# chngdickson/ov2slam

Measured on AMD Instinct MI355X. Metric: tracked_frames_per_sec, higher is better.
Workload: dtype u8/s16 fixed-point + f32

## Files before the change

include/ov2slam_hip.h:

```cpp
#ifndef OV2SLAM_HIP_H
#define OV2SLAM_HIP_H

#include <stddef.h>
#include <stdint.h>

#ifdef __cplusplus
extern "C" {
#endif

typedef int ov2_status;
enum {
    OV2_OK = 0,
    OV2_ERR_INVALID = -1,
    OV2_ERR_HIP = -2,
    OV2_ERR_NOMEM = -3,
    OV2_ERR_NODEVICE = -4,
    OV2_ERR_UNSUPPORTED = -5
};

typedef struct ov2_ctx ov2_ctx;
typedef struct ov2_images ov2_images;
typedef struct ov2_pyr ov2_pyr;

ov2_status ov2_ctx_create(int device, ov2_ctx **out);
// ... 55 lines not shown
                            int max_iter, float eps, float err_th, float fb_th, int n, const float *kps_xy,
                            float *priors_xy, uint8_t *status);
ov2_status ov2_klt_track_fb_dev(ov2_ctx *ctx, const ov2_pyr *prev, const ov2_pyr *cur, int win, int nlevels,
                                int max_iter, float eps, float err_th, float fb_th, int n, const float *d_kps_xy,
                                float *d_priors_xy, uint8_t *d_status, const int32_t *d_img_idx,
                                uint32_t *d_iters);

ov2_status ov2_klt_tracking_frame_dev(ov2_ctx *ctx, const ov2_pyr *prev, const ov2_pyr *cur, int win,
                                      int nlevels_full, int max_iter, float eps, float err_th, float fb_th, int n,
                                      const float *d_kps_xy, const float *d_prior_xy, const uint8_t *d_has_prior,
                                      const int32_t *d_img_idx, float *d_out_xy, uint8_t *d_out_status,
                                      int32_t *d_p3p_req , uint32_t *d_iters );

ov2_status ov2_klt_set_lanes(ov2_ctx *ctx, int lanes);
ov2_status ov2_klt_set_stereo_split(ov2_ctx *ctx, int k);

ov2_status ov2_line_min_sad(ov2_ctx *ctx, const ov2_pyr *left, const ov2_pyr *right, int level, int nwinsize, int go_left,
                            int n, const float *pts_xy, float *xprior, float *l1err);
ov2_status ov2_line_min_sad_dev(ov2_ctx *ctx, const ov2_pyr *left, const ov2_pyr *right, int level, int nwinsize,
                                int go_left, int n, const float *d_pts_xy, const int32_t *d_img_idx, float *d_xprior,
                                float *d_l1err);

typedef struct ov2_cam_model {
    double K[4];
    int32_t model;
    int32_t n_coeffs;
    double D[5];
} ov2_cam_model;

ov2_status ov2_stereo_matching(ov2_ctx *ctx, const ov2_pyr *left, const ov2_pyr *right, int win, int nlevels_full,
// ... 539 lines not shown
```

ov2slam_amd/_lib.py:

```python
import ctypes as C
import os

_HERE = os.path.dirname(os.path.abspath(__file__))
LIB_PATH = os.environ.get("OV2SLAM_HIP_LIB") or os.path.join(_HERE, "lib", "libov2hip.so")

vp = C.c_void_p
vpp = C.POINTER(C.c_void_p)
ip = C.POINTER(C.c_int)
fp = C.POINTER(C.c_float)

SIGNATURES = {
    "ov2_ctx_create": (C.c_int, [C.c_int, vpp]),
    "ov2_ctx_create_ex": (C.c_int, [C.c_int, C.c_int, vpp]),
    "ov2_ctx_destroy": (None, [vp]),
    "ov2_last_error": (C.c_char_p, [vp]),
    "ov2_status_string": (C.c_char_p, [C.c_int]),
    "ov2_ctx_synchronize": (C.c_int, [vp]),
    "ov2_ctx_set_kf_overlap": (C.c_int, [vp, C.c_int]),
    "ov2_ctx_set_kf_lazy_join": (C.c_int, [vp, C.c_int]),
    "ov2_ctx_get_kf_lazy_join": (C.c_int, [vp]),
    "ov2_ctx_kf_join_stats": (C.c_int, [vp, C.POINTER(C.c_int64)]),
    "ov2_kf_ranges_independent": (C.c_int, [C.POINTER(C.c_size_t), C.c_int, C.POINTER(C.c_size_t), C.c_int,
                                            C.POINTER(C.c_size_t), C.c_int, C.POINTER(C.c_size_t), C.c_int]),
    "ov2_ctx_set_wave_prio": (C.c_int, [vp, C.c_int]),
# ... 25 lines not shown
    "ov2_pyr_retain": (None, [vp]),
    "ov2_pyr_release": (None, [vp]),
    "ov2_pyr_release_from": (None, [vp, vp]),
    "ov2_pyr_batch": (C.c_int, [vp]),
    "ov2_pyr_nlevels": (C.c_int, [vp]),
    "ov2_pyr_level_size": (C.c_int, [vp, C.c_int, ip, ip, ip]),
    "ov2_pyr_download_level": (C.c_int, [vp, vp, C.c_int, C.c_int, vp, vp]),
    "ov2_klt_track_fb": (C.c_int, [vp, vp, vp, C.c_int, C.c_int, C.c_int, C.c_float, C.c_float, C.c_float,
                                   C.c_int, vp, vp, vp]),
    "ov2_klt_track_fb_dev": (C.c_int, [vp, vp, vp, C.c_int, C.c_int, C.c_int, C.c_float, C.c_float, C.c_float,
                                       C.c_int, vp, vp, vp, vp, vp]),
    "ov2_klt_tracking_frame_dev": (C.c_int, [vp, vp, vp, C.c_int, C.c_int, C.c_int, C.c_float, C.c_float,
                                             C.c_float, C.c_int, vp, vp, vp, vp, vp, vp, vp, vp]),
    "ov2_klt_set_lanes": (C.c_int, [vp, C.c_int]),
    "ov2_klt_set_stereo_split": (C.c_int, [vp, C.c_int]),
    "ov2_line_min_sad": (C.c_int, [vp, vp, vp, C.c_int, C.c_int, C.c_int, C.c_int, vp, vp, vp]),
    "ov2_line_min_sad_dev": (C.c_int, [vp, vp, vp, C.c_int, C.c_int, C.c_int, C.c_int, vp, vp, vp, vp]),
    "ov2_stereo_matching": (C.c_int, [vp, vp, vp, C.c_int, C.c_int, C.c_int, C.c_float, C.c_float, C.c_float, C.c_int,
                                      vp, vp, vp, vp, C.c_int, vp, vp, vp, vp]),
    "ov2_stereo_matching_dev": (C.c_int, [vp, vp, vp, C.c_int, C.c_int, C.c_int, C.c_float, C.c_float, C.c_float, C.c_int,
                                          vp, vp, vp, vp, vp, C.c_int, vp, vp, vp, vp, vp]),
    "ov2_detect_grid": (C.c_int, [vp, vp, C.c_int, C.c_int, C.c_int, C.POINTER(C.c_double), C.c_int, vp, vp, C.c_int, ip, vp]),
    "ov2_detect_grid_batch": (C.c_int, [vp, vp, C.c_int, C.c_int, C.POINTER(C.c_double), ip, vp, vp, C.c_int, ip, vp, C.c_int]),
    "ov2_detect_grid_batch_dev": (C.c_int, [vp, vp, C.c_int, C.c_int, vp, C.c_int, vp, vp, vp, vp, C.c_int, vp, vp, C.c_int]),
    "ov2_fast_detect_batch": (C.c_int, [vp, vp, C.c_int, C.c_int, vp, vp, C.c_int, C.c_int, vp, vp, vp, vp]),
    "ov2_fast_detect_batch_dev": (C.c_int, [vp, vp, C.c_int, C.c_int, C.c_int, vp, vp, C.c_int, C.c_int, vp, vp, vp, vp]),
    "ov2_ba_default_options": (None, [vp, C.c_float]),
    "ov2_ba_solve": (C.c_int, [vp, vp, vp, vp]),
    "ov2_ba_solve_batch": (C.c_int, [vp, C.c_int, vp, vp, vp]),
    "ov2_ba_solve_batch_dev": (C.c_int, [vp, C.c_int, vp, vp, vp]),
# ... 120 lines not shown
```

ov2slam_amd/csrc/ctx.hip:

```cpp
#include "ov2_internal.h"

#include <cstdlib>

ov2_status ov2_set_err(ov2_ctx *ctx, ov2_status s, const char *fmt, ...)
{
    char buf[512];
    va_list ap;
    va_start(ap, fmt);
    vsnprintf(buf, sizeof(buf), fmt, ap);
    va_end(ap);
    if (ctx) {
        std::lock_guard<std::mutex> g(ctx->mu);
        ctx->err = buf;
    }
    return s;
}

extern "C" const char *ov2_status_string(ov2_status s)
{
    switch (s) {
    case OV2_OK: return "ok";
    case OV2_ERR_INVALID: return "invalid argument";
    case OV2_ERR_HIP: return "HIP runtime error";
    case OV2_ERR_NOMEM: return "out of memory";
// ... 99 lines not shown
        for (int x = 0; x < OV2_CU_MASK_XCDS; ++x) {
            int bits = 0, own = 0;
            for (int k = x; k < total; k += OV2_CU_MASK_XCDS, ++own) bits += (int)(mask[k >> 5] >> (k & 31) & 1u);
            effective_cus += bits ? bits : own;
        }
    }
    ov2_ctx *c = new ov2_ctx();
    c->device = device;
    c->scratch_dev = nullptr;
    c->scratch_bytes = 0;
    c->tmp_img = nullptr;
    c->ktime_on = false;
    c->wave_prio = high_priority ? OV2_WAVE_PRIO_HIGH : 0;
    c->klt_lanes = 0;
    c->klt_stereo_split = -1;
    c->knn_lanes = 0;
    c->knn_cus = effective_cus;
    c->cu_share = n_cus;
    c->cu_layout = layout;
    c->counts_as_high = false;
    c->lcd_splits = 0;
    c->lcd_calls = 0;
    c->ba_arena = nullptr;
    c->ba_arena_cap = 0;
    c->ba_host = nullptr;
    c->ba_host_cap = 0;
    c->ba_copy_stream = nullptr;
    c->klt_counts[0] = c->klt_counts[1] = nullptr;
    c->klt_counts_words = 0;
    c->klt_counts_cur = 0;
// ... 555 lines not shown
```

ov2slam_amd/csrc/klt.hip:

```cpp
#include <cstdlib>

#include "ov2_internal.h"
#include "ov2_wave.h"

using namespace ov2wave;

namespace {

struct klt_params {
    int win, nlevels, max_iter;
    int wave_prio;
    double eps2;
    float err_th;
    double fb_th;
    float min_eig_thr;
    int rule33;
};

#define W_BITS 14

__device__ __forceinline__ void lk_weights(float a, float b, int &w00, int &w01, int &w10, int &w11)
{
    w00 = (int)__builtin_rintf((1.f - a) * (1.f - b) * (float)(1 << W_BITS));
    w01 = (int)__builtin_rintf(a * (1.f - b) * (float)(1 << W_BITS));
    w10 = (int)__builtin_rintf((1.f - a) * b * (float)(1 << W_BITS));
    w11 = (1 << W_BITS) - w00 - w01 - w10;
}

__device__ __forceinline__ unsigned ld_u16(const unsigned char *p)
{
    unsigned short r;
    __builtin_memcpy(&r, p, 2);
// ... 423 lines not shown
    }
}
template <int B, int NB>
__device__ __forceinline__ void klt3_stage_region(const level_ptrs &J, int rr0, int cc0, int c, bool store, unsigned char *lj)
{
    if constexpr (B < NB) {
        constexpr int T0 = klt3::NLD * B / NB, T1 = klt3::NLD * (B + 1) / NB;
        klt3_segs<T0, T1> S;
        klt3_load_region(J, rr0, cc0, c, S);
        klt3_store_region(S, c, store, lj);
        __builtin_amdgcn_sched_barrier(0);
        klt3_stage_region<B + 1, NB>(J, rr0, cc0, c, store, lj);
    }
}

template <int WIN>
__device__ __forceinline__ int lk_level3(const level_ptrs &I, const level_ptrs &J, int pad, int level, int max_level,
                                         bool run, float kx, float ky, float &nx_io, float &ny_io, int &status,
                                         float &err, const klt_params &P, int c, bool lane_ok, unsigned &passes,
                                         unsigned char *lj)
{
    static_assert(WIN == 9, "three lanes x three columns");
#ifdef KLT3_VGPR_CLAIM
    asm volatile("" ::: KLT3_VGPR_CLAIM);
#endif
    constexpr int NPX = 3 * WIN, NQ = (NPX + 1) / 2;
    const float FLT_SCALE = 1.f / (float)(1 << 20);
    const float half = (float)(WIN - 1) * 0.5f;
    const float lscale = __builtin_ldexpf(1.f, -level);
    float px = kx * lscale, py = ky * lscale;
    float nx, ny;
    if (level == max_level) { nx = nx_io * lscale; ny = ny_io * lscale; }
    else { nx = nx_io * 2.f; ny = ny_io * 2.f; }
    if (run) { nx_io = nx; ny_io = ny; }

    px -= half; py -= half;
    const int ipx = (int)floorf(px), ipy = (int)floorf(py);
    if (run && (ipx < -WIN || ipx >= I.w || ipy < -WIN || ipy >= I.h)) {
        if (level == 0) { status = 0; err = 0.f; }
        run = false;
    }
    if (!__any(run)) return 0;
    if (run) passes += 1u;
    int w00, w01, w10, w11;
    lk_weights(px - (float)ipx, py - (float)ipy, w00, w01, w10, w11);

    unsigned Iv2[NQ], Ix2[NQ], Iy2[NQ];
    int sA11 = 0, sA12 = 0, sA22 = 0;
    int rr0, cc0;
    {
        const float sx = nx - half, sy = ny - half;
        const int inx0 = (int)floorf(sx), iny0 = (int)floorf(sy);
        const bool in0 = run && !(inx0 < -WIN || inx0 >= J.w || iny0 < -WIN || iny0 >= J.h);
        klt3_region_origin(J, pad, in0 ? inx0 : 0, in0 ? iny0 : 0, rr0, cc0);
        const int bx0 = (run ? (OV2_LM + ipx) : OV2_LM) + 3 * c, by = run ? (ipy + pad) : pad;
        const int ax = bx0 - 1;
        const unsigned io = I.img_o + (unsigned)(by * I.istride + (ax & ~3));
        const unsigned shI = (unsigned)ax & 3u;
        struct row3 { unsigned x, y, z; };
        row3 irow[WIN + 3];
#define KLT3_LOAD_ROW(p)                                                                                                  \
    do {                                                                                                                  \
        const int dr = (p) == 0 ? (by > 0 ? -1 : 0) : ((p) == WIN + 2 ? (by + WIN + 1 < I.rows ? WIN + 1 : WIN) : (p) - 1); \
        __builtin_memcpy(&irow[p], __builtin_assume_aligned(I.base + (size_t)(io + (unsigned)(dr * I.istride)), 4), 12);   \
    } while (0)
        constexpr int R1 = 6;
// ... 89 lines not shown
    float D = A11 * A22 - A12 * A12;
    const float min_eig = __fdiv_rn(A22 + A11 - __fsqrt_rn((A11 - A22) * (A11 - A22) + 4.f * A12 * A12),
                                    (float)(2 * WIN * WIN));
    if (run) {
        err = min_eig;
        if (min_eig < P.min_eig_thr || D < 1.1920929e-07f ) {
            if (level == 0) status = 0;
            run = false;
        }
    }
    D = __fdiv_rn(1.f, D);

    nx -= half; ny -= half;
    float pdx = 0.f, pdy = 0.f;
    int iters = 0;
    for (int j = 0; j < P.max_iter; ++j) {
        if (!__any(run)) break;
        const int inx = (int)floorf(nx), iny = (int)floorf(ny);
        if (run && (inx < -WIN || inx >= J.w || iny < -WIN || iny >= J.h)) {
            if (level == 0) status = 0;
            run = false;
        }
        int w00j, w01j, w10j, w11j;
        lk_weights(nx - (float)inx, ny - (float)iny, w00j, w01j, w10j, w11j);
        int rb = run ? iny + pad - rr0 : 0, cb = run ? OV2_LM + inx - cc0 : 0;
        const bool out = (unsigned)rb > (unsigned)klt3::ROW_SPAN || (unsigned)cb > (unsigned)klt3::COL_SPAN;
        if (__any(out)) {
            __syncthreads();
            if (out) {
                klt3_region_origin(J, pad, inx, iny, rr0, cc0);
                klt3_stage_region<0, KLT3_REGION_BATCHES>(J, rr0, cc0, c, lane_ok, lj);
                rb = iny + pad - rr0; cb = OV2_LM + inx - cc0;
// ... 34 lines not shown
        float b1, b2;
        if (__all((unsigned)(pb1 + (1 << 27)) < (1u << 28) && (unsigned)(pb2 + (1 << 27)) < (1u << 28))) {
            b1 = (float)sum3_i32(pb1, c) * FLT_SCALE;
            b2 = (float)sum3_i32(pb2, c) * FLT_SCALE;
        } else {
            b1 = (float)sum3_f64((double)pb1, c) * FLT_SCALE;
            b2 = (float)sum3_f64((double)pb2, c) * FLT_SCALE;
        }
        const float dx = (A12 * b2 - A22 * b1) * D;
        const float dy = (A12 * b1 - A11 * b2) * D;
        if (run) {
            ++iters;
            nx += dx; ny += dy;
            nx_io = nx + half; ny_io = ny + half;
            if ((double)dx * dx + (double)dy * dy <= P.eps2) run = false;
            else if (j > 0 && fabsf(dx + pdx) <= 0.01f && fabsf(dy + pdy) <= 0.01f) {
                nx_io -= dx * 0.5f; ny_io -= dy * 0.5f;
                run = false;
            }
            pdx = dx; pdy = dy;
        }
    }
    return iters;
}

template <int WIN, int GL>
__device__ __forceinline__ int lk_pass(const level_ptrs &I, const level_ptrs &J, int pad, int level, int max_level, bool run,
                                       float kx, float ky, float &nx_io, float &ny_io, int &status, float &err,
                                       const klt_params &P, int sub, bool lane_ok, unsigned &passes, unsigned char *smem, int slot)
{
    if constexpr (GL == 3) {
        return lk_level3<WIN>(I, J, pad, level, max_level, run, kx, ky, nx_io, ny_io, status, err, P, sub, lane_ok, passes,
                              smem + slot * klt3::RSZ);
    } else {
        constexpr int KPW = 64 / GL, WB = klt_lds<WIN>::WB, GB = klt_lds<WIN>::GB;
        return lk_level<WIN, GL>(I, J, pad, level, max_level, run, kx, ky, nx_io, ny_io, status, err, P, sub, passes,
                                 smem + slot * WB, smem + KPW * WB + slot * WB, smem + 2 * KPW * WB + slot * GB);
    }
}

struct __attribute__((aligned(16))) klt_handover { float fx, fy, err; unsigned work; };

template <int WIN, int GL>
__device__ __forceinline__ int fb_track(const ov2_pyr_view &pv, const ov2_pyr_view &cv, int b, bool act, float kx,
                                          float ky, float &fx, float &fy, const klt_params &P, int nlevels, int sub,
                                          bool lane_ok, unsigned &work, unsigned char *smem, int slot,
                                          int l_hi, int l_lo, float err0, unsigned work0, float &err_out)
{
    int status = 1;
    float err = err0;
    unsigned it = work0 & 0xffffu, passes = work0 >> 16;
    for (int l = l_hi; l >= l_lo; --l) {
        const level_ptrs I = level_of(pv, l, b), J = level_of(cv, l, b);
        it += lk_pass<WIN, GL>(I, J, pv.pad, l, nlevels, act, kx, ky, fx, fy, status, err, P, sub, lane_ok, passes, smem, slot);
    }
    if (l_lo > 0) {
        work = it | (passes << 16);
        err_out = err;
        return 0;
    }
    const int W0 = cv.lv[0].w, H0 = cv.lv[0].h;
    int ok = act && status && !(err > P.err_th) &&
             (1.f <= fx && fx < (float)W0 - 1.f && 1.f <= fy && fy < (float)H0 - 1.f);
    int st2 = 1;
    float e2 = 0.f, bx = kx, by = ky;
    {
        const level_ptrs I = level_of(cv, 0, b), J = level_of(pv, 0, b);
        it += lk_pass<WIN, GL>(I, J, cv.pad, 0, 0, ok != 0, fx, fy, bx, by, st2, e2, P, sub, lane_ok, passes, smem, slot);
    }
    if (ok) {
        if (!st2) ok = 0;
        else {
            const float dx = kx - bx, dy = ky - by;
            const double nrm = __dsqrt_rn((double)dx * dx + (double)dy * dy);
            if (nrm > P.fb_th) ok = 0;
        }
    }
    work = it | (passes << 16);
    return ok;
}

template <int WIN, int GL>
__device__ __forceinline__ int fb_track(const ov2_pyr_view &pv, const ov2_pyr_view &cv, int b, bool act, float kx,
                                          float ky, float &fx, float &fy, const klt_params &P, int nlevels, int sub,
                                          bool lane_ok, unsigned &work, unsigned char *smem, int slot)
{
    float err;
    return fb_track<WIN, GL>(pv, cv, b, act, kx, ky, fx, fy, P, nlevels, sub, lane_ok, work, smem, slot, nlevels, 0, 0.f, 0u, err);
}

#define KLT_GL8_MIN_KPS 65536
#ifndef KLT_STEREO_SPLIT_DEFAULT
#define KLT_STEREO_SPLIT_DEFAULT 0
#endif
#ifndef KLT_SPLIT_C_FIRST
#define KLT_SPLIT_C_FIRST 1
#endif
#ifndef KLT_WAVE_CAP
#define KLT_WAVE_CAP 4
#endif
#ifndef KLT3_WAVE_MIN
#define KLT3_WAVE_MIN 2
#endif
#define KLT_WAVES(W, G) ((G) == 3 ? KLT3_WAVE_MIN : 1), ((G) == 3 ? KLT3_WAVES : KLT_WAVE_CAP)

template <int WIN, int KLT_GL>
__global__ __launch_bounds__(64) __attribute__((amdgpu_waves_per_eu(KLT_WAVES(WIN, KLT_GL)))) void klt_fb_kernel(ov2_pyr_view pv, ov2_pyr_view cv, klt_params P, int n,
                                                    const float2 *__restrict__ kps, float2 *__restrict__ priors,
// ... 80 lines not shown
        out_status[i] = (unsigned char)ok;
        if (iters) iters[is_a ? i : n + i] = work;
        if (is_a) atomicAdd(&counts[64 * b + (i & 63)], 1u + ((unsigned)ok << 16));
    }
    const bool retry = mine && is_a && !ok;
    const unsigned long long rm = __ballot(retry);
    if (rm) {
        const int lane = (int)threadIdx.x, leader = __ffsll((long long)rm) - 1;
        int base = 0;
        if (lane == leader) base = (int)atomicAdd(&cnt[2], (unsigned)__popcll(rm));
        base = __shfl(base, leader);
        if (retry) list_c[base + __popcll(rm & ((1ull << lane) - 1ull))] = i;
    }
}

template <int WIN, int KLT_GL, bool SPLIT>
__global__ __launch_bounds__(64) __attribute__((amdgpu_waves_per_eu(KLT_WAVES(WIN, KLT_GL)))) void klt_stage1_kernel(ov2_pyr_view pv, ov2_pyr_view cv, klt_params P, int n,
                                                        const float2 *__restrict__ kps,
                                                        const float2 *__restrict__ prior,
                                                        const int *__restrict__ img_idx, float2 *__restrict__ out_xy,
                                                        unsigned char *__restrict__ out_status,
                                                        unsigned *__restrict__ counts ,
                                                        unsigned *__restrict__ iters, const int *__restrict__ list_a,
                                                        const int *__restrict__ list_b, unsigned *__restrict__ cnt,
                                                        int *__restrict__ list_c,
                                                        int b_word ,
                                                        int split_k ,
                                                        klt_handover *__restrict__ hand )
{
    __shared__ __attribute__((aligned(16))) unsigned char smem[klt_smem<WIN, KLT_GL>::BYTES];
    using M = klt_map<KLT_GL>;
// ... 4 lines not shown
    const int g = is_a ? (int)blockIdx.x - groups_b : (int)blockIdx.x;
    const int total = is_a ? total_a : total_b;
    if (g * KLT_KPW >= total) return;
    ov2wave::set_wave_prio(P.wave_prio);
    const int slot = M::slot((int)threadIdx.x), sub = M::sub((int)threadIdx.x), idx = g * KLT_KPW + slot;
    const bool lane_ok = M::lane_ok((int)threadIdx.x);
    const bool act = idx < total && lane_ok;
    const int i = (is_a ? list_a : list_b)[idx < total ? idx : total - 1];
    const float2 kp = kps[i];
    const int b = img_idx ? img_idx[i] : 0;
    float2 pr = (is_a || !P.rule33) ? prior[i] : kp;
    unsigned work = 0;
    const int nl = is_a ? min(1, pv.nlevels - 1) : P.nlevels;
    const bool upper = SPLIT && !is_a;
    float err;
    const int ok = fb_track<WIN, KLT_GL>(pv, cv, b, act, kp.x, kp.y, pr.x, pr.y, P, nl, sub, lane_ok, work, smem, slot, nl,
                                         upper ? split_k + 1 : 0, 0.f, 0u, err);
    if (upper) {
        if (act && sub == 0) hand[i] = klt_handover{pr.x, pr.y, err, work};
        return;
    }
    klt_stage1_finish(act && sub == 0, is_a, i, b, n, ok, pr, work, out_xy, out_status, counts, iters, cnt, list_c);
}

template <int WIN, int KLT_GL>
__global__ __launch_bounds__(64) __attribute__((amdgpu_waves_per_eu(KLT_WAVES(WIN, KLT_GL)))) void klt_stage2_kernel(ov2_pyr_view pv, ov2_pyr_view cv, klt_params P, int n,
                                                        const float2 *__restrict__ kps,
                                                        const int *__restrict__ img_idx, float2 *__restrict__ out_xy,
                                                        unsigned char *__restrict__ out_status,
                                                        const unsigned *__restrict__ counts, int *__restrict__ p3p_req,
                                                        unsigned *__restrict__ iters, const int *__restrict__ list_c,
                                                        const unsigned *__restrict__ cnt, int batch,
                                                        unsigned *__restrict__ next_counts, int next_words,
                                                        const int *__restrict__ list_b, int b_word,
                                                        const float2 *__restrict__ prior,
                                                        int split_k ,
                                                        const klt_handover *__restrict__ hand)
{
    __shared__ __attribute__((aligned(16))) unsigned char smem[klt_smem<WIN, KLT_GL>::BYTES];
    using M = klt_map<KLT_GL>;
    constexpr int KLT_KPW = M::KPW;
    const int slot = M::slot((int)threadIdx.x), sub = M::sub((int)threadIdx.x);
    const bool lane_ok = M::lane_ok((int)threadIdx.x);
    for (int q = blockIdx.x * 64 + threadIdx.x; q < next_words; q += gridDim.x * 64) next_counts[q] = 0u;
    auto tally = [&](int b, int &n3, int &good) {
        n3 = 0; good = 0;
        if constexpr (KLT_GL == 3) {
            for (int q = sub; q < 64; q += 3) {
                const unsigned cw = counts[64 * b + q];
                n3 += (int)(cw & 0xffffu); good += (int)(cw >> 16);
            }
            n3 = sum3_i32(n3, sub); good = sum3_i32(good, sub);
        } else {
            for (int q = 0; q < 64 / KLT_GL; ++q) {
                const unsigned cw = counts[64 * b + sub * (64 / KLT_GL) + q];
                n3 += (int)(cw & 0xffffu); good += (int)(cw >> 16);
            }
            n3 = row_sum_i32<KLT_GL>(n3); good = row_sum_i32<KLT_GL>(good);
        }
    };
    if (p3p_req && P.rule33) {
        for (int b0 = blockIdx.x * KLT_KPW; b0 < batch; b0 += gridDim.x * KLT_KPW) {
            const int b = b0 + slot;
            int n3, good;
            tally(min(b, batch - 1), n3, good);
            if (b < batch && lane_ok && sub == 0 && n3 > 0 && (double)good < 0.33 * (double)n3) p3p_req[b] = 1;
        }
    }
    const int total_b = (int)cnt[b_word], total_c = (int)cnt[2];
    const bool b_first = split_k < 0 || !KLT_SPLIT_C_FIRST;
    const int groups_1 = ((b_first ? total_b : total_c) + KLT_KPW - 1) / KLT_KPW;
    const bool first = (int)blockIdx.x < groups_1;
    const bool is_b = first == b_first;
    const int g = first ? (int)blockIdx.x : (int)blockIdx.x - groups_1;
    const int total = is_b ? total_b : total_c;
    if (g * KLT_KPW >= total) return;
    ov2wave::set_wave_prio(P.wave_prio);
    const int idx = g * KLT_KPW + slot;
    const bool act = idx < total && lane_ok;
    const int i = (is_b ? list_b : list_c)[idx < total ? idx : total - 1];
    const int b = img_idx ? img_idx[i] : 0;
    const float2 kp = kps[i];
    float2 pr;
    int l_hi = P.nlevels;
    float err0 = 0.f;
    unsigned work0 = 0;
    if (is_b) {
        if (split_k >= 0) {
            const klt_handover hr = hand[i];
            pr = make_float2(hr.fx, hr.fy);
            err0 = hr.err; work0 = hr.work; l_hi = split_k;
        } else {
            pr = prior[i];
        }
    } else {
        int n3, good;
        tally(b, n3, good);
        const bool drop = P.rule33 && n3 > 0 && (double)good < 0.33 * (double)n3;
        pr = drop ? kp : out_xy[i];
    }
    unsigned work = 0;
    float err;
    const int ok = fb_track<WIN, KLT_GL>(pv, cv, b, act, kp.x, kp.y, pr.x, pr.y, P, P.nlevels, sub, lane_ok, work, smem, slot,
                                         l_hi, 0, err0, work0, err);
    if (act && sub == 0) {
        out_xy[i] = pr;
        out_status[i] = (unsigned char)ok;
        if (iters) iters[n + i] = work;
    }
}

int klt_lanes_for(const ov2_ctx *c, int n, int win, const ov2_pyr *a, const ov2_pyr *b)
{
    static const int env = [] { const char *e = getenv("OV2_KLT_LANES"); return e ? atoi(e) : 0; }();
    const int forced = c->klt_lanes ? c->klt_lanes : env;
    const bool fits32 = a->buf->bytes < (1ull << 32) && b->buf->bytes < (1ull << 32);
    if (forced == 8 || forced == 16 || (forced == 3 && win == 9 && fits32)) return forced;
    if (win == 9 && fits32) return 3;
    return n >= KLT_GL8_MIN_KPS ? 8 : 16;
// ... 11 lines not shown
        return ov2_set_err(c, OV2_ERR_INVALID, "win=%d unsupported (odd, 3..11, <= pyramid pad %d)", win, a.pad);
    if (nlevels < 0) return ov2_set_err(c, OV2_ERR_INVALID, "nlevels < 0");
    if (a.nlevels < nlevels + 1) nlevels = a.nlevels - 1;
    P->win = win;
    P->wave_prio = c->wave_prio;
    P->nlevels = nlevels;
    P->max_iter = max_iter < 0 ? 0 : (max_iter > 100 ? 100 : max_iter);
    double e = (double)eps;
    if (e < 0.) e = 0.;
    if (e > 10.) e = 10.;
    P->eps2 = e * e;
    P->err_th = err_th;
    P->fb_th = (double)fb_th;
    P->min_eig_thr = 1e-4f;
    P->rule33 = 1;
    return OV2_OK;
}

}

extern "C" ov2_status ov2_klt_set_lanes(ov2_ctx *c, int lanes)
{
    if (!c) return OV2_ERR_INVALID;
    if (lanes != 0 && lanes != 3 && lanes != 8 && lanes != 16) return ov2_set_err(c, OV2_ERR_INVALID, "lanes per keypoint: 0 (auto), 3, 8 or 16");
    c->klt_lanes = lanes;
    return OV2_OK;
}

extern "C" ov2_status ov2_klt_set_stereo_split(ov2_ctx *c, int k)
{
    if (!c) return OV2_ERR_INVALID;
    c->klt_stereo_split = k < 0 ? -1 : k;
    return OV2_OK;
}

extern "C" ov2_status ov2_klt_track_fb_dev(ov2_ctx *c, const ov2_pyr *prev, const ov2_pyr *cur, int win, int nlevels,
                                           int max_iter, float eps, float err_th, float fb_th, int n,
                                           const float *d_kps, float *d_priors, uint8_t *d_status,
                                           const int32_t *d_img_idx, uint32_t *d_iters)
{
    if (!c) return OV2_ERR_INVALID;
    if (n == 0) return OV2_OK;
    if (n < 0 || !d_kps || !d_priors || !d_status) return ov2_set_err(c, OV2_ERR_INVALID, "null/negative argument");
    klt_params P;
    ov2_status s = make_params(c, prev, cur, win, nlevels, max_iter, eps, err_th, fb_th, &P);
    if (s != OV2_OK) return s;
    OV2_HIP(c, hipSetDevice(c->device));
// ... 68 lines not shown
    if (n == 0) return OV2_OK;
    if (n < 0 || !d_kps || !d_prior || !d_has_prior || !d_out_xy || !d_out_status)
        return ov2_set_err(c, OV2_ERR_INVALID, "null/negative argument");
    klt_params P;
    ov2_status s = make_params(c, prev, cur, win, nlevels_full, max_iter, eps, err_th, fb_th, &P);
    if (s != OV2_OK) return s;
    P.rule33 = rule33 ? 1 : 0;
    OV2_HIP(c, hipSetDevice(c->device));
    if ((s = ov2_pyr_wait_ready(c, prev)) != OV2_OK || (s = ov2_pyr_wait_ready(c, cur)) != OV2_OK) return s;
    const int lanes = klt_lanes_for(c, n, win, prev, cur);
    if (lanes != 3 && ((s = ov2_pyr_need_grad(c, prev)) != OV2_OK || (s = ov2_pyr_need_grad(c, cur)) != OV2_OK)) return s;
    const int B = prev->buf->batch;
    const size_t cnt_words = (size_t)B * 64 + 16;
    if (cnt_words > c->klt_counts_words) {
        OV2_HIP(c, hipStreamSynchronize(c->stream));
        for (int i = 0; i < 2; ++i) {
            if (c->klt_counts[i]) OV2_HIP(c, hipFree(c->klt_counts[i]));
            c->klt_counts[i] = nullptr;
        }
        c->klt_counts_words = 0;
        const size_t words = cnt_words + cnt_words / 2;
        for (int i = 0; i < 2; ++i) OV2_HIP(c, hipMalloc((void **)&c->klt_counts[i], words * sizeof(unsigned)));
        c->klt_counts_words = words;
        c->klt_counts_dirty = true;
    }
    if (c->klt_counts_dirty)
        for (int i = 0; i < 2; ++i) OV2_HIP(c, hipMemsetAsync(c->klt_counts[i], 0, c->klt_counts_words * sizeof(unsigned), c->stream));
    c->klt_counts_dirty = true;
    void *scr = nullptr;
    const size_t lists_bytes = (3 * (size_t)n * sizeof(int) + 255) / 256 * 256;
    s = ov2_scratch(c, lists_bytes + (size_t)n * sizeof(klt_handover) + 256, &scr);
    if (s != OV2_OK) return s;
    unsigned *counts = c->klt_counts[c->klt_counts_cur], *live_cnt = counts + (size_t)B * 64;
    unsigned *next_counts = c->klt_counts[c->klt_counts_cur ^ 1];
    const int next_words = (int)c->klt_counts_words;
    int *list_a = (int *)scr, *list_b = list_a + n, *list_c = list_b + n;
    const size_t N = (size_t)n;
    const ov2_byte_range kf_rd[4] = {ov2_range(d_kps, 8 * N), ov2_range(d_prior, 8 * N), ov2_range(d_has_prior, N), ov2_range(d_img_idx, 4 * N)};
    const ov2_byte_range kf_wr[4] = {ov2_range(d_out_xy, 8 * N), ov2_range(d_out_status, N), ov2_range(d_p3p_req, sizeof(int32_t) * (size_t)B),
                                     ov2_range(d_iters, 8 * N)};
    const hipStream_t ms = ov2_kf_stream_for(c, true, kf_rd, 4, kf_wr, 4);
    if (c->kf.want_stereo_ev) {
        OV2_HIP(c, hipEventRecord(c->kf.fork, c->stream.h));
        c->kf.want_stereo_ev = false;
    }
    const dim3 cgrid((n + KLT_COMPACT_KPWG - 1) / KLT_COMPACT_KPWG);
    const int want_k = c->klt_stereo_split < 0 ? KLT_STEREO_SPLIT_DEFAULT : c->klt_stereo_split;
    const int split_k = (!P.rule33 && want_k < P.nlevels) ? want_k : -1;
    const int b_word1 = (P.rule33 || split_k >= 0) ? 1 : 3, b_word2 = P.rule33 ? 3 : 1;
    klt_handover *hand = reinterpret_cast<klt_handover *>((char *)scr + lists_bytes);
#define KLT_STAGES_GL(W, G)                                                                                     \
    do {                                                                                                        \
         \
        const dim3 tgrid((n + klt_map<G>::KPW - 1) / klt_map<G>::KPW + 2);                                      \
        OV2_LAUNCH_ON(c, OV2_K_DETECT + 4, ms, klt_compact_kernel, cgrid, dim3(256), 0, ms, n, d_has_prior,     \
                   d_iters, list_a, list_b, live_cnt, d_p3p_req, B, P.wave_prio);                               \
        if (split_k >= 0)                                                                                       \
            OV2_LAUNCH_ON(c, OV2_K_KLT_STAGE1, ms, (klt_stage1_kernel<W, G, true>), tgrid, dim3(64), 0, ms,     \
                       prev->buf->view, cur->buf->view, P, n, reinterpret_cast<const float2 *>(d_kps),          \
                       reinterpret_cast<const float2 *>(d_prior), d_img_idx, reinterpret_cast<float2 *>(d_out_xy), \
                       d_out_status, counts, d_iters, list_a, list_b, live_cnt, list_c, b_word1, split_k, hand); \
        else                                                                                                    \
            OV2_LAUNCH_ON(c, OV2_K_KLT_STAGE1, ms, (klt_stage1_kernel<W, G, false>), tgrid, dim3(64), 0, ms,    \
                       prev->buf->view, cur->buf->view, P, n, reinterpret_cast<const float2 *>(d_kps),          \
                       reinterpret_cast<const float2 *>(d_prior), d_img_idx, reinterpret_cast<float2 *>(d_out_xy), \
                       d_out_status, counts, d_iters, list_a, list_b, live_cnt, list_c, b_word1, split_k, hand); \
        OV2_LAUNCH_ON(c, OV2_K_KLT_STAGE2, ms, (klt_stage2_kernel<W, G>), tgrid, dim3(64), 0, ms,               \
                   prev->buf->view, cur->buf->view, P, n, reinterpret_cast<const float2 *>(d_kps), d_img_idx,   \
                   reinterpret_cast<float2 *>(d_out_xy), d_out_status, counts, d_p3p_req, d_iters, list_c,      \
                   live_cnt, B, next_counts, next_words, list_b, b_word2,                                       \
                   reinterpret_cast<const float2 *>(d_prior), split_k, hand);                                   \
    } while (0)
#define KLT_STAGES(W)                                                                                           \
    do {                                                                                                        \
        if (lanes == 8) KLT_STAGES_GL(W, 8);                                                                       \
        else KLT_STAGES_GL(W, 16);                                                                              \
    } while (0)
    switch (win) {
    case 3: KLT_STAGES(3); break;
    case 5: KLT_STAGES(5); break;
    case 7: KLT_STAGES(7); break;
    case 9:
        if (lanes == 3) KLT_STAGES_GL(9, 3);
        else KLT_STAGES(9);
        break;
    default: KLT_STAGES(11); break;
    }
#undef KLT_STAGES
#undef KLT_STAGES_GL
    OV2_HIP(c, hipGetLastError());
    c->klt_counts_cur ^= 1;
    c->klt_counts_dirty = false;
    return OV2_OK;
}
```

ov2slam_amd/csrc/ov2_internal.h:

```cpp
#pragma once
#include <hip/hip_runtime.h>

#include <atomic>
#include <cstdarg>
#include <cstdio>
#include <cstring>
#include <mutex>
#include <string>
#include <vector>

#include "../../include/ov2slam_hip.h"

#define OV2_MAX_LEVELS 8
#define OV2_LM 16

struct ov2_level_desc {
    int w, h;
    int istride;
    int gstride;
    int rows;
    size_t img_off;
    size_t grad_off;
    size_t img_bstride;
    size_t grad_bstride;
// ... 154 lines not shown
    void *lpg_dev;
    size_t lpg_dev_cap;
    void *ba_arena2;
    size_t ba_arena2_cap;
    void *ba_host;
    size_t ba_host_cap;
    unsigned *klt_counts[2];
    size_t klt_counts_words;
    int klt_counts_cur;
    bool klt_counts_dirty;
    hipStream_t ba_copy_stream;
    hipEvent_t ba_copy_ev[2];
    int wave_prio;
    int klt_lanes;
    int klt_stereo_split;
    int knn_lanes;
    int knn_cus;
    int cu_share, cu_layout;
    bool counts_as_high;
    int lcd_splits;
    long long lcd_calls;
    std::vector<struct ov2_lcd_table *> lcd_tables;
    bool ktime_on;
    std::vector<ov2_ktime_rec> ktime_recs;
    std::vector<hipEvent_t> ktime_free;
};

struct ov2_images {
    ov2_ctx *ctx;
    int batch, w, h;
// ... 54 lines not shown
```

ov2slam_amd/frontend.py:

```python
import ctypes as C

import numpy as np

from . import _lib


WAVE_PRIO_HIGH = 2


CU_LAYOUT_SPREAD, CU_LAYOUT_PACKED = 0, 1
CU_MASK_XCDS = 8


def cu_mask_build(total_cus, n_cus, layout=CU_LAYOUT_SPREAD):
    out = (C.c_uint32 * ((int(total_cus) + 31) // 32 if total_cus > 0 else 1))()
    st = _lib.load().ov2_cu_mask_build(int(total_cus), int(n_cus), int(layout), out)
    if st != 0:
        raise _lib.Ov2Error(f"ov2_cu_mask_build({total_cus}, {n_cus}, {layout}): status {st}")
    return np.array(out, np.uint32)


def _check(ctx_handle, status):
    if status != 0:
        lib = _lib.load()
# ... 19 lines not shown
        self.h = h

    def close(self):
        if getattr(self, "h", None):
            self.lib.ov2_ctx_destroy(self.h)
            self.h = None

    def __del__(self):
        self.close()

    def set_klt_lanes(self, lanes):
        _check(self.h, self.lib.ov2_klt_set_lanes(self.h, int(lanes)))

    def set_stereo_split(self, k):
        _check(self.h, self.lib.ov2_klt_set_stereo_split(self.h, int(k)))

    def set_knn_lanes(self, lanes):
        _check(self.h, self.lib.ov2_knn_set_lanes(self.h, int(lanes)))

    def set_kf_overlap(self, on):
        _check(self.h, self.lib.ov2_ctx_set_kf_overlap(self.h, int(bool(on))))

    def set_wave_prio(self, level):
        _check(self.h, self.lib.ov2_ctx_set_wave_prio(self.h, int(level)))

    def get_wave_prio(self):
        return int(self.lib.ov2_ctx_get_wave_prio(self.h))

    def get_cu_share(self):
        return int(self.lib.ov2_ctx_get_cu_share(self.h))
# ... 361 lines not shown
```

Baseline: 309,500.

## Park straggler KLT lanes in split stereo descent and resume them compacted

In the split two-stage KLT path, a wave whose live keypoint count drops to a threshold after k iterations saves each lane's iteration state to a park record. Those keypoints are appended to a new compacted list, and stage 2 launches extra 'D' waves that resume them at the saved level and iteration. The aim is to stop nearly empty waves from running long Lucas-Kanade tails at low occupancy. In exchange it adds per-keypoint park records, atomics, extra stage-2 groups and per-level park counters, plus an env knob and stats API.

```diff
diff --git a/include/ov2slam_hip.h b/include/ov2slam_hip.h
--- a/include/ov2slam_hip.h
+++ b/include/ov2slam_hip.h
@@ -93,6 +93,8 @@
 
 ov2_status ov2_klt_set_lanes(ov2_ctx *ctx, int lanes);
 ov2_status ov2_klt_set_stereo_split(ov2_ctx *ctx, int k);
+ov2_status ov2_klt_set_stereo_park(ov2_ctx *ctx, int k, int t);
+ov2_status ov2_ctx_klt_park_stats(ov2_ctx *ctx, int64_t out[10]);
 
 ov2_status ov2_line_min_sad(ov2_ctx *ctx, const ov2_pyr *left, const ov2_pyr *right, int level, int nwinsize, int go_left,
                             int n, const float *pts_xy, float *xprior, float *l1err);
diff --git a/ov2slam_amd/_lib.py b/ov2slam_amd/_lib.py
--- a/ov2slam_amd/_lib.py
+++ b/ov2slam_amd/_lib.py
@@ -63,6 +63,8 @@
                                              C.c_float, C.c_int, vp, vp, vp, vp, vp, vp, vp, vp]),
     "ov2_klt_set_lanes": (C.c_int, [vp, C.c_int]),
     "ov2_klt_set_stereo_split": (C.c_int, [vp, C.c_int]),
+    "ov2_klt_set_stereo_park": (C.c_int, [vp, C.c_int, C.c_int]),
+    "ov2_ctx_klt_park_stats": (C.c_int, [vp, C.POINTER(C.c_int64)]),
     "ov2_line_min_sad": (C.c_int, [vp, vp, vp, C.c_int, C.c_int, C.c_int, C.c_int, vp, vp, vp]),
     "ov2_line_min_sad_dev": (C.c_int, [vp, vp, vp, C.c_int, C.c_int, C.c_int, C.c_int, vp, vp, vp, vp]),
     "ov2_stereo_matching": (C.c_int, [vp, vp, vp, C.c_int, C.c_int, C.c_int, C.c_float, C.c_float, C.c_float, C.c_int,
diff --git a/ov2slam_amd/csrc/ctx.hip b/ov2slam_amd/csrc/ctx.hip
--- a/ov2slam_amd/csrc/ctx.hip
+++ b/ov2slam_amd/csrc/ctx.hip
@@ -137,6 +137,17 @@
     c->wave_prio = high_priority ? OV2_WAVE_PRIO_HIGH : 0;
     c->klt_lanes = 0;
     c->klt_stereo_split = -1;
+    c->klt_park_k = c->klt_park_t = -1;
+    if (const char *park_env = getenv("OV2_KLT_STEREO_PARK")) {
+        int k = -1, t = -1;
+        const int got = sscanf(park_env, "%d,%d", &k, &t);
+        if (got >= 1 && !(k > 0 && got == 2 && t == 0)) {
+            c->klt_park_k = k < 0 ? -1 : (k > 100 ? 100 : k);
+            c->klt_park_t = (k < 0 || got < 2 || t < 0) ? -1 : (t > 21 ? 21 : t);
+        }
+    }
+    for (auto &v : c->klt_park_folded) v = 0;
+    c->klt_park_calls = 0;
     c->knn_lanes = 0;
     c->knn_cus = effective_cus;
     c->cu_share = n_cus;
diff --git a/ov2slam_amd/csrc/klt.hip b/ov2slam_amd/csrc/klt.hip
--- a/ov2slam_amd/csrc/klt.hip
+++ b/ov2slam_amd/csrc/klt.hip
@@ -12,10 +12,13 @@
     int wave_prio;
     double eps2;
     float err_th;
+    short park_k, park_t;
     double fb_th;
     float min_eig_thr;
     int rule33;
 };
+
+static_assert(sizeof(klt_params) == 48, "klt_params: the kernels' argument layout");
 
 #define W_BITS 14
 
@@ -469,11 +472,34 @@
     }
 }
 
-template <int WIN>
+struct __attribute__((aligned(8))) klt_park_rec {
+    float nx, ny;
+    float nx_io, ny_io;
+    float pdx, pdy;
+    float err;
+    unsigned work;
+    int level, j;
+};
+#define KLT_HAND_PARKED 0xffffffffu
+#define KLT_CNT_D 4
+#define KLT_CNT_PARKED 8
+#define KLT_PARK_WORDS 16
+static_assert(OV2_MAX_LEVELS + 1 <= KLT_PARK_WORDS, "parked per level + D waves");
+static_assert(KLT_CNT_PARKED + OV2_MAX_LEVELS <= 16, "the list-length block has 16 words");
+struct klt_park_io {
+    klt_park_rec *rec;
+    unsigned *level_cnt;
+    unsigned it;
+    int level;
+    bool on;
+    bool parked;
+};
+
+template <int WIN, int PM = 0>
 __device__ __forceinline__ int lk_level3(const level_ptrs &I, const level_ptrs &J, int pad, int level, int max_level,
                                          bool run, float kx, float ky, float &nx_io, float &ny_io, int &status,
                                          float &err, const klt_params &P, int c, bool lane_ok, unsigned &passes,
-                                         unsigned char *lj)
+                                         unsigned char *lj, klt_park_io &pk)
 {
     static_assert(WIN == 9, "three lanes x three columns");
 #ifdef KLT3_VGPR_CLAIM
@@ -487,7 +513,9 @@
     float nx, ny;
     if (level == max_level) { nx = nx_io * lscale; ny = ny_io * lscale; }
     else { nx = nx_io * 2.f; ny = ny_io * 2.f; }
-    if (run) { nx_io = nx; ny_io = ny; }
+    bool res = false;
+    if constexpr (PM == 2) res = run && level == pk.level;
+    if (run && !res) { nx_io = nx; ny_io = ny; }
 
     px -= half; py -= half;
     const int ipx = (int)floorf(px), ipy = (int)floorf(py);
@@ -496,7 +524,7 @@
         run = false;
     }
     if (!__any(run)) return 0;
-    if (run) passes += 1u;
+    if (run && !res) passes += 1u;
     int w00, w01, w10, w11;
     lk_weights(px - (float)ipx, py - (float)ipy, w00, w01, w10, w11);
 
@@ -504,7 +532,10 @@
     int sA11 = 0, sA12 = 0, sA22 = 0;
     int rr0, cc0;
     {
-        const float sx = nx - half, sy = ny - half;
+        float sx = nx - half, sy = ny - half;
+        if constexpr (PM == 2) {
+            if (res) { sx = pk.rec->nx; sy = pk.rec->ny; }
+        }
         const int inx0 = (int)floorf(sx), iny0 = (int)floorf(sy);
         const bool in0 = run && !(inx0 < -WIN || inx0 >= J.w || iny0 < -WIN || iny0 >= J.h);
         klt3_region_origin(J, pad, in0 ? inx0 : 0, in0 ? iny0 : 0, rr0, cc0);
@@ -624,8 +655,32 @@
     nx -= half; ny -= half;
     float pdx = 0.f, pdy = 0.f;
     int iters = 0;
+    int j0 = 0;
+    if constexpr (PM == 2) {
+        if (res) {
+            const klt_park_rec r = *pk.rec;
+            nx = r.nx; ny = r.ny; pdx = r.pdx; pdy = r.pdy; j0 = r.j;
+        }
+    }
     for (int j = 0; j < P.max_iter; ++j) {
+        if constexpr (PM == 2) {
+            if (j + j0 >= P.max_iter) run = false;
+        }
         if (!__any(run)) break;
+        if constexpr (PM == 1) {
+            if (pk.on && j >= (int)P.park_k) {
+                const unsigned long long live = __ballot(run && c == 0 && lane_ok);
+                if (__popcll(live) <= (int)P.park_t) {
+                    if (run) {
+                        if (c == 0)
+                            *pk.rec = klt_park_rec{nx, ny, nx_io, ny_io, pdx, pdy, err, (pk.it + (unsigned)iters) | (passes << 16), level, j};
+                        pk.parked = true;
+                    }
+                    if ((int)threadIdx.x == __ffsll((long long)live) - 1) atomicAdd(&pk.level_cnt[level], (unsigned)__popcll(live));
+                    break;
+                }
+            }
+        }
         const int inx = (int)floorf(nx), iny = (int)floorf(ny);
         if (run && (inx < -WIN || inx >= J.w || iny < -WIN || iny >= J.h)) {
             if (level == 0) status = 0;
@@ -690,7 +745,7 @@
             nx += dx; ny += dy;
             nx_io = nx + half; ny_io = ny + half;
             if ((double)dx * dx + (double)dy * dy <= P.eps2) run = false;
-            else if (j > 0 && fabsf(dx + pdx) <= 0.01f && fabsf(dy + pdy) <= 0.01f) {
+            else if ((PM == 2 ? j + j0 : j) > 0 && fabsf(dx + pdx) <= 0.01f && fabsf(dy + pdy) <= 0.01f) {
                 nx_io -= dx * 0.5f; ny_io -= dy * 0.5f;
                 run = false;
             }
@@ -700,15 +755,17 @@
     return iters;
 }
 
-template <int WIN, int GL>
+template <int WIN, int GL, int PM = 0>
 __device__ __forceinline__ int lk_pass(const level_ptrs &I, const level_ptrs &J, int pad, int level, int max_level, bool run,
                                        float kx, float ky, float &nx_io, float &ny_io, int &status, float &err,
-                                       const klt_params &P, int sub, bool lane_ok, unsigned &passes, unsigned char *smem, int slot)
+                                       const klt_params &P, int sub, bool lane_ok, unsigned &passes, unsigned char *smem, int slot,
+                                       klt_park_io &pk)
 {
     if constexpr (GL == 3) {
-        return lk_level3<WIN>(I, J, pad, level, max_level, run, kx, ky, nx_io, ny_io, status, err, P, sub, lane_ok, passes,
-                              smem + slot * klt3::RSZ);
+        return lk_level3<WIN, PM>(I, J, pad, level, max_level, run, kx, ky, nx_io, ny_io, status, err, P, sub, lane_ok, passes,
+                                  smem + slot * klt3::RSZ, pk);
     } else {
+        static_assert(PM == 0, "parking is the three-lane mapping's");
         constexpr int KPW = 64 / GL, WB = klt_lds<WIN>::WB, GB = klt_lds<WIN>::GB;
         return lk_level<WIN, GL>(I, J, pad, level, max_level, run, kx, ky, nx_io, ny_io, status, err, P, sub, passes,
                                  smem + slot * WB, smem + KPW * WB + slot * WB, smem + 2 * KPW * WB + slot * GB);
@@ -717,18 +774,22 @@
 
 struct __attribute__((aligned(16))) klt_handover { float fx, fy, err; unsigned work; };
 
-template <int WIN, int GL>
+template <int WIN, int GL, int PM = 0>
 __device__ __forceinline__ int fb_track(const ov2_pyr_view &pv, const ov2_pyr_view &cv, int b, bool act, float kx,
                                           float ky, float &fx, float &fy, const klt_params &P, int nlevels, int sub,
                                           bool lane_ok, unsigned &work, unsigned char *smem, int slot,
-                                          int l_hi, int l_lo, float err0, unsigned work0, float &err_out)
+                                          int l_hi, int l_lo, float err0, unsigned work0, float &err_out, klt_park_io &pk)
 {
     int status = 1;
     float err = err0;
     unsigned it = work0 & 0xffffu, passes = work0 >> 16;
+    klt_park_io none{};
     for (int l = l_hi; l >= l_lo; --l) {
         const level_ptrs I = level_of(pv, l, b), J = level_of(cv, l, b);
-        it += lk_pass<WIN, GL>(I, J, pv.pad, l, nlevels, act, kx, ky, fx, fy, status, err, P, sub, lane_ok, passes, smem, slot);
+        bool run = act;
+        if constexpr (PM == 1) { run = act && !pk.parked; pk.it = it; }
+        if constexpr (PM == 2) run = act && (pk.level < 0 || l <= pk.level);
+        it += lk_pass<WIN, GL, PM>(I, J, pv.pad, l, nlevels, run, kx, ky, fx, fy, status, err, P, sub, lane_ok, passes, smem, slot, pk);
     }
     if (l_lo > 0) {
         work = it | (passes << 16);
@@ -742,7 +803,7 @@
     float e2 = 0.f, bx = kx, by = ky;
     {
         const level_ptrs I = level_of(cv, 0, b), J = level_of(pv, 0, b);
-        it += lk_pass<WIN, GL>(I, J, cv.pad, 0, 0, ok != 0, fx, fy, bx, by, st2, e2, P, sub, lane_ok, passes, smem, slot);
+        it += lk_pass<WIN, GL>(I, J, cv.pad, 0, 0, ok != 0, fx, fy, bx, by, st2, e2, P, sub, lane_ok, passes, smem, slot, none);
     }
     if (ok) {
         if (!st2) ok = 0;
@@ -762,12 +823,19 @@
                                           bool lane_ok, unsigned &work, unsigned char *smem, int slot)
 {
     float err;
-    return fb_track<WIN, GL>(pv, cv, b, act, kx, ky, fx, fy, P, nlevels, sub, lane_ok, work, smem, slot, nlevels, 0, 0.f, 0u, err);
+    klt_park_io none{};
+    return fb_track<WIN, GL>(pv, cv, b, act, kx, ky, fx, fy, P, nlevels, sub, lane_ok, work, smem, slot, nlevels, 0, 0.f, 0u, err, none);
 }
 
 #define KLT_GL8_MIN_KPS 65536
 #ifndef KLT_STEREO_SPLIT_DEFAULT
 #define KLT_STEREO_SPLIT_DEFAULT 0
+#endif
+#ifndef KLT_STEREO_PARK_K_DEFAULT
+#define KLT_STEREO_PARK_K_DEFAULT 4
+#endif
+#ifndef KLT_STEREO_PARK_T_DEFAULT
+#define KLT_STEREO_PARK_T_DEFAULT 4
 #endif
 #ifndef KLT_SPLIT_C_FIRST
 #define KLT_SPLIT_C_FIRST 1
@@ -878,7 +946,7 @@
     }
 }
 
-template <int WIN, int KLT_GL, bool SPLIT>
+template <int WIN, int KLT_GL, bool SPLIT, bool PARK = false>
 __global__ __launch_bounds__(64) __attribute__((amdgpu_waves_per_eu(KLT_WAVES(WIN, KLT_GL)))) void klt_stage1_kernel(ov2_pyr_view pv, ov2_pyr_view cv, klt_params P, int n,
                                                         const float2 *__restrict__ kps,
                                                         const float2 *__restrict__ prior,
@@ -913,16 +981,36 @@
     const int nl = is_a ? min(1, pv.nlevels - 1) : P.nlevels;
     const bool upper = SPLIT && !is_a;
     float err;
-    const int ok = fb_track<WIN, KLT_GL>(pv, cv, b, act, kp.x, kp.y, pr.x, pr.y, P, nl, sub, lane_ok, work, smem, slot, nl,
-                                         upper ? split_k + 1 : 0, 0.f, 0u, err);
+    klt_park_io pk{};
+    if constexpr (PARK) {
+        static_assert(SPLIT && KLT_GL == 3, "parking belongs to the split descent of the three-lane mapping");
+        pk.rec = reinterpret_cast<klt_park_rec *>(hand + n) + i;
+        pk.level_cnt = cnt + KLT_CNT_PARKED;
+        pk.on = upper && P.park_k > 0;
+    }
+    const int ok = fb_track<WIN, KLT_GL, PARK ? 1 : 0>(pv, cv, b, act, kp.x, kp.y, pr.x, pr.y, P, nl, sub, lane_ok, work, smem, slot, nl,
+                                                       upper ? split_k + 1 : 0, 0.f, 0u, err, pk);
     if (upper) {
-        if (act && sub == 0) hand[i] = klt_handover{pr.x, pr.y, err, work};
+        if constexpr (PARK) {
+            const bool mine = act && sub == 0;
+            if (mine) hand[i] = klt_handover{pr.x, pr.y, err, pk.parked ? KLT_HAND_PARKED : work};
+            const unsigned long long dm = __ballot(mine && pk.parked);
+            if (dm) {
+                const int lane = (int)threadIdx.x, leader = __ffsll((long long)dm) - 1;
+                int base = 0;
+                if (lane == leader) base = (int)atomicAdd(&cnt[KLT_CNT_D], (unsigned)__popcll(dm));
+                base = __shfl(base, leader);
+                if (mine && pk.parked) (list_c + n)[base + __popcll(dm & ((1ull << lane) - 1ull))] = i;
+            }
+        } else {
+            if (act && sub == 0) hand[i] = klt_handover{pr.x, pr.y, err, work};
+        }
         return;
     }
     klt_stage1_finish(act && sub == 0, is_a, i, b, n, ok, pr, work, out_xy, out_status, counts, iters, cnt, list_c);
 }
 
-template <int WIN, int KLT_GL>
+template <int WIN, int KLT_GL, bool PARK = false>
 __global__ __launch_bounds__(64) __attribute__((amdgpu_waves_per_eu(KLT_WAVES(WIN, KLT_GL)))) void klt_stage2_kernel(ov2_pyr_view pv, ov2_pyr_view cv, klt_params P, int n,
                                                         const float2 *__restrict__ kps,
                                                         const int *__restrict__ img_idx, float2 *__restrict__ out_xy,
@@ -941,6 +1029,14 @@
     constexpr int KLT_KPW = M::KPW;
     const int slot = M::slot((int)threadIdx.x), sub = M::sub((int)threadIdx.x);
     const bool lane_ok = M::lane_ok((int)threadIdx.x);
+    if constexpr (PARK) {
+        static_assert(KLT_GL == 3, "parking belongs to the three-lane mapping");
+        if (blockIdx.x == 0 && threadIdx.x <= OV2_MAX_LEVELS) {
+            const int q = (int)threadIdx.x;
+            const unsigned v = q < OV2_MAX_LEVELS ? cnt[KLT_CNT_PARKED + q] : (cnt[KLT_CNT_D] + KLT_KPW - 1) / KLT_KPW;
+            if (v) atomicAdd(&next_counts[next_words + q], v);
+        }
+    }
     for (int q = blockIdx.x * 64 + threadIdx.x; q < next_words; q += gridDim.x * 64) next_counts[q] = 0u;
     auto tally = [&](int b, int &n3, int &good) {
         n3 = 0; good = 0;
@@ -967,28 +1063,48 @@
         }
     }
     const int total_b = (int)cnt[b_word], total_c = (int)cnt[2];
-    const bool b_first = split_k < 0 || !KLT_SPLIT_C_FIRST;
-    const int groups_1 = ((b_first ? total_b : total_c) + KLT_KPW - 1) / KLT_KPW;
-    const bool first = (int)blockIdx.x < groups_1;
-    const bool is_b = first == b_first;
-    const int g = first ? (int)blockIdx.x : (int)blockIdx.x - groups_1;
-    const int total = is_b ? total_b : total_c;
+    bool is_b, is_d = false;
+    int g, total;
+    if constexpr (PARK) {
+        const int total_d = (int)cnt[KLT_CNT_D];
+        const int groups_c = (total_c + KLT_KPW - 1) / KLT_KPW, groups_d = (total_d + KLT_KPW - 1) / KLT_KPW;
+        const int bid = (int)blockIdx.x;
+        is_d = bid >= groups_c && bid < groups_c + groups_d;
+        is_b = bid >= groups_c + groups_d;
+        g = is_b ? bid - groups_c - groups_d : (is_d ? bid - groups_c : bid);
+        total = is_b ? total_b : (is_d ? total_d : total_c);
+    } else {
+        const bool b_first = split_k < 0 || !KLT_SPLIT_C_FIRST;
+        const int groups_1 = ((b_first ? total_b : total_c) + KLT_KPW - 1) / KLT_KPW;
+        const bool first = (int)blockIdx.x < groups_1;
+        is_b = first == b_first;
+        g = first ? (int)blockIdx.x : (int)blockIdx.x - groups_1;
+        total = is_b ? total_b : total_c;
+    }
     if (g * KLT_KPW >= total) return;
     ov2wave::set_wave_prio(P.wave_prio);
     const int idx = g * KLT_KPW + slot;
-    const bool act = idx < total && lane_ok;
-    const int i = (is_b ? list_b : list_c)[idx < total ? idx : total - 1];
+    bool act = idx < total && lane_ok;
+    const int i = (is_b ? list_b : (is_d ? list_c + n : list_c))[idx < total ? idx : total - 1];
     const int b = img_idx ? img_idx[i] : 0;
     const float2 kp = kps[i];
     float2 pr;
     int l_hi = P.nlevels;
     float err0 = 0.f;
     unsigned work0 = 0;
-    if (is_b) {
+    klt_park_io pk{};
+    pk.level = -1;
+    if (PARK && is_d) {
+        pk.rec = const_cast<klt_park_rec *>(reinterpret_cast<const klt_park_rec *>(hand + n)) + i;
+        const klt_park_rec r = *pk.rec;
+        pr = make_float2(r.nx_io, r.ny_io);
+        err0 = r.err; work0 = r.work; pk.level = r.level;
+    } else if (is_b) {
         if (split_k >= 0) {
             const klt_handover hr = hand[i];
             pr = make_float2(hr.fx, hr.fy);
             err0 = hr.err; work0 = hr.work; l_hi = split_k;
+            if (PARK && hr.work == KLT_HAND_PARKED) act = false;
         } else {
             pr = prior[i];
         }
@@ -1000,8 +1116,8 @@
     }
     unsigned work = 0;
     float err;
-    const int ok = fb_track<WIN, KLT_GL>(pv, cv, b, act, kp.x, kp.y, pr.x, pr.y, P, P.nlevels, sub, lane_ok, work, smem, slot,
-                                         l_hi, 0, err0, work0, err);
+    const int ok = fb_track<WIN, KLT_GL, PARK ? 2 : 0>(pv, cv, b, act, kp.x, kp.y, pr.x, pr.y, P, P.nlevels, sub, lane_ok, work, smem, slot,
+                                                       l_hi, 0, err0, work0, err, pk);
     if (act && sub == 0) {
         out_xy[i] = pr;
         out_status[i] = (unsigned char)ok;
@@ -1043,6 +1159,18 @@
     P->fb_th = (double)fb_th;
     P->min_eig_thr = 1e-4f;
     P->rule33 = 1;
+    P->park_k = P->park_t = 0;
+    return OV2_OK;
+}
+
+ov2_status klt_park_totals(ov2_ctx *c, int64_t acc[OV2_MAX_LEVELS + 1])
+{
+    for (int i = 0; i < 2; ++i) {
+        if (!c->klt_counts[i] || !c->klt_counts_words) continue;
+        unsigned dev[OV2_MAX_LEVELS + 1];
+        OV2_HIP(c, hipMemcpy(dev, c->klt_counts[i] + c->klt_counts_words, sizeof(dev), hipMemcpyDeviceToHost));
+        for (int q = 0; q <= OV2_MAX_LEVELS; ++q) acc[q] += dev[q];
+    }
     return OV2_OK;
 }
 
@@ -1060,6 +1188,29 @@
 {
     if (!c) return OV2_ERR_INVALID;
     c->klt_stereo_split = k < 0 ? -1 : k;
+    return OV2_OK;
+}
+
+extern "C" ov2_status ov2_klt_set_stereo_park(ov2_ctx *c, int k, int t)
+{
+    if (!c) return OV2_ERR_INVALID;
+    if (k > 0 && t == 0) return ov2_set_err(c, OV2_ERR_INVALID, "stereo park: t = 0 keypoints can never park (k = 0 switches parking off)");
+    c->klt_park_k = k < 0 ? -1 : (k > 100 ? 100 : k);
+    c->klt_park_t = (k < 0 || t < 0) ? -1 : (t > klt_map<3>::KPW ? klt_map<3>::KPW : t);
+    return OV2_OK;
+}
+
+extern "C" ov2_status ov2_ctx_klt_park_stats(ov2_ctx *c, int64_t out[2 + OV2_MAX_LEVELS])
+{
+    if (!c || !out) return OV2_ERR_INVALID;
+    ov2_status s = ov2_ctx_synchronize(c);
+    if (s != OV2_OK) return s;
+    int64_t tot[OV2_MAX_LEVELS + 1];
+    for (int q = 0; q <= OV2_MAX_LEVELS; ++q) tot[q] = c->klt_park_folded[q];
+    if ((s = klt_park_totals(c, tot)) != OV2_OK) return s;
+    out[0] = c->klt_park_calls;
+    out[1] = tot[OV2_MAX_LEVELS];
+    for (int l = 0; l < OV2_MAX_LEVELS; ++l) out[2 + l] = tot[l];
     return OV2_OK;
 }
 
@@ -1158,13 +1309,17 @@
     const size_t cnt_words = (size_t)B * 64 + 16;
     if (cnt_words > c->klt_counts_words) {
         OV2_HIP(c, hipStreamSynchronize(c->stream));
+        if ((s = klt_park_totals(c, c->klt_park_folded)) != OV2_OK) return s;
         for (int i = 0; i < 2; ++i) {
             if (c->klt_counts[i]) OV2_HIP(c, hipFree(c->klt_counts[i]));
             c->klt_counts[i] = nullptr;
         }
         c->klt_counts_words = 0;
         const size_t words = cnt_words + cnt_words / 2;
-        for (int i = 0; i < 2; ++i) OV2_HIP(c, hipMalloc((void **)&c->klt_counts[i], words * sizeof(unsigned)));
+        for (int i = 0; i < 2; ++i) {
+            OV2_HIP(c, hipMalloc((void **)&c->klt_counts[i], (words + KLT_PARK_WORDS) * sizeof(unsigned)));
+            OV2_HIP(c, hipMemsetAsync(c->klt_counts[i] + words, 0, KLT_PARK_WORDS * sizeof(unsigned), c->stream));
+        }
         c->klt_counts_words = words;
         c->klt_counts_dirty = true;
     }
@@ -1172,8 +1327,8 @@
         for (int i = 0; i < 2; ++i) OV2_HIP(c, hipMemsetAsync(c->klt_counts[i], 0, c->klt_counts_words * sizeof(unsigned), c->stream));
     c->klt_counts_dirty = true;
     void *scr = nullptr;
-    const size_t lists_bytes = (3 * (size_t)n * sizeof(int) + 255) / 256 * 256;
-    s = ov2_scratch(c, lists_bytes + (size_t)n * sizeof(klt_handover) + 256, &scr);
+    const size_t lists_bytes = (4 * (size_t)n * sizeof(int) + 255) / 256 * 256;
+    s = ov2_scratch(c, lists_bytes + (size_t)n * (sizeof(klt_handover) + sizeof(klt_park_rec)) + 256, &scr);
     if (s != OV2_OK) return s;
     unsigned *counts = c->klt_counts[c->klt_counts_cur], *live_cnt = counts + (size_t)B * 64;
     unsigned *next_counts = c->klt_counts[c->klt_counts_cur ^ 1];
@@ -1193,7 +1348,13 @@
     const int split_k = (!P.rule33 && want_k < P.nlevels) ? want_k : -1;
     const int b_word1 = (P.rule33 || split_k >= 0) ? 1 : 3, b_word2 = P.rule33 ? 3 : 1;
     klt_handover *hand = reinterpret_cast<klt_handover *>((char *)scr + lists_bytes);
-#define KLT_STAGES_GL(W, G)                                                                                     \
+    const int want_pk = c->klt_park_k < 0 ? KLT_STEREO_PARK_K_DEFAULT : c->klt_park_k;
+    const int want_pt = c->klt_park_t < 0 ? KLT_STEREO_PARK_T_DEFAULT : c->klt_park_t;
+    const bool park = split_k >= 0 && lanes == 3 && win == 9 && want_pk > 0 && want_pt > 0;
+    if (park) {
+        P.park_k = (short)want_pk; P.park_t = (short)want_pt;
+    }
+#define KLT_STAGES_GL(W, G)                                                                                   \
     do {                                                                                                        \
          \
         const dim3 tgrid((n + klt_map<G>::KPW - 1) / klt_map<G>::KPW + 2);                                      \
@@ -1215,6 +1376,23 @@
                    live_cnt, B, next_counts, next_words, list_b, b_word2,                                       \
                    reinterpret_cast<const float2 *>(d_prior), split_k, hand);                                   \
     } while (0)
+#define KLT_STAGES_PARK()                                                                                       \
+    do {                                                                                                        \
+        const int ng = (n + klt_map<3>::KPW - 1) / klt_map<3>::KPW;                                             \
+        const dim3 tgrid(ng + 2), tgrid2(2 * ng + 2);                                                           \
+        OV2_LAUNCH_ON(c, OV2_K_DETECT + 4, ms, klt_compact_kernel, cgrid, dim3(256), 0, ms, n, d_has_prior,     \
+                   d_iters, list_a, list_b, live_cnt, d_p3p_req, B, P.wave_prio);                               \
+        OV2_LAUNCH_ON(c, OV2_K_KLT_STAGE1, ms, (klt_stage1_kernel<9, 3, true, true>), tgrid, dim3(64), 0, ms,   \
+                   prev->buf->view, cur->buf->view, P, n, reinterpret_cast<const float2 *>(d_kps),              \
+                   reinterpret_cast<const float2 *>(d_prior), d_img_idx, reinterpret_cast<float2 *>(d_out_xy),  \
+                   d_out_status, counts, d_iters, list_a, list_b, live_cnt, list_c, b_word1, split_k, hand);    \
+        OV2_LAUNCH_ON(c, OV2_K_KLT_STAGE2, ms, (klt_stage2_kernel<9, 3, true>), tgrid2, dim3(64), 0, ms,        \
+                   prev->buf->view, cur->buf->view, P, n, reinterpret_cast<const float2 *>(d_kps), d_img_idx,   \
+                   reinterpret_cast<float2 *>(d_out_xy), d_out_status, counts, d_p3p_req, d_iters, list_c,      \
+                   live_cnt, B, next_counts, next_words, list_b, b_word2,                                       \
+                   reinterpret_cast<const float2 *>(d_prior), split_k, hand);                                   \
+        ++c->klt_park_calls;                                                                                    \
+    } while (0)
 #define KLT_STAGES(W)                                                                                           \
     do {                                                                                                        \
         if (lanes == 8) KLT_STAGES_GL(W, 8);                                                                       \
@@ -1225,11 +1403,13 @@
     case 5: KLT_STAGES(5); break;
     case 7: KLT_STAGES(7); break;
     case 9:
-        if (lanes == 3) KLT_STAGES_GL(9, 3);
+        if (park) KLT_STAGES_PARK();
+        else if (lanes == 3) KLT_STAGES_GL(9, 3);
         else KLT_STAGES(9);
         break;
     default: KLT_STAGES(11); break;
     }
+#undef KLT_STAGES_PARK
 #undef KLT_STAGES
 #undef KLT_STAGES_GL
     OV2_HIP(c, hipGetLastError());
diff --git a/ov2slam_amd/csrc/ov2_internal.h b/ov2slam_amd/csrc/ov2_internal.h
--- a/ov2slam_amd/csrc/ov2_internal.h
+++ b/ov2slam_amd/csrc/ov2_internal.h
@@ -192,6 +192,9 @@
     int wave_prio;
     int klt_lanes;
     int klt_stereo_split;
+    int klt_park_k, klt_park_t;
+    int64_t klt_park_folded[OV2_MAX_LEVELS + 1];
+    int64_t klt_park_calls;
     int knn_lanes;
     int knn_cus;
     int cu_share, cu_layout;
diff --git a/ov2slam_amd/frontend.py b/ov2slam_amd/frontend.py
--- a/ov2slam_amd/frontend.py
+++ b/ov2slam_amd/frontend.py
@@ -57,6 +57,14 @@
 
     def set_stereo_split(self, k):
         _check(self.h, self.lib.ov2_klt_set_stereo_split(self.h, int(k)))
+
+    def set_stereo_park(self, k, t=-1):
+        _check(self.h, self.lib.ov2_klt_set_stereo_park(self.h, int(k), int(t)))
+
+    def klt_park_stats(self):
+        out = (C.c_int64 * 10)()
+        _check(self.h, self.lib.ov2_ctx_klt_park_stats(self.h, out))
+        return dict(calls=int(out[0]), d_waves=int(out[1]), parked=[int(v) for v in out[2:]])
 
     def set_knn_lanes(self, lanes):
         _check(self.h, self.lib.ov2_knn_set_lanes(self.h, int(lanes)))
```

Measured after the change: 293,300. 0.948x the previous value.
